# FofanovLab/mtsv_tools

Hardware: AMD Instinct MI355X
Metric: reads/sec (whole node), 150bp reads vs MG-index (higher is better)
Workload: dtype u32/i16

## Files before the change

### include/mtsv_amd.h

```cpp
#ifndef MTSV_AMD_H
#define MTSV_AMD_H

#include <stddef.h>
#include <stdint.h>

#ifdef __cplusplus
extern "C" {
#endif

#define MTSV_OK 0
#define MTSV_E_ARG (-1)
#define MTSV_E_IO (-2)
#define MTSV_E_FORMAT (-3)
#define MTSV_E_DEVICE (-4)
#define MTSV_E_LIMIT (-5)
#define MTSV_E_NOMEM (-6)

typedef struct mtsv_index mtsv_index;
typedef struct mtsv_batch mtsv_batch;

typedef struct {
    double edit_rate;
    uint32_t seed_size;
    uint32_t seed_interval;
// ... 21 lines not shown
    uint64_t sa_s;
    uint64_t file_bytes;
    uint64_t device_bytes;
    uint32_t kmer_k;
    uint32_t sa_full;
} mtsv_index_info_t;

#define MTSV_N_STAGES 8
typedef struct {
    float stage_ms[MTSV_N_STAGES];
    uint64_t n_reads;
    uint64_t n_seed_slots;
    uint64_t n_seed_hits;
    uint64_t lf_steps;
    uint64_t n_candidates;
    uint64_t n_verified;
    uint64_t window_bytes;
    uint64_t n_hits;
    uint64_t n_passes;
    uint64_t n_rounds;
    uint64_t n_lanes;
    uint64_t sw_cell_pairs;
    float sw_prefilter_ms;
    float sw_sweep_ms;
    uint64_t n_sw_passed;
    float sw_diag_ms;
    float sw_bound_ms;
    float edit_ms;
    uint64_t myers_columns;
    uint64_t n_sw_bound_refuted;
    uint64_t verify_turns;
    uint64_t verify_lanes_max;
    uint64_t myers_grid_max;
} mtsv_batch_stats;

const char *mtsv_last_error(void);
const char *mtsv_version(void);
void mtsv_params_default(mtsv_params *p);

int mtsv_device_count(void);

int mtsv_index_load(const char *path, mtsv_index **out);
int mtsv_index_build(uint64_t n_seqs, const uint32_t *tax_ids, const uint32_t *gis,
                     const uint8_t *const *seqs, const uint64_t *seq_lens, uint32_t occ_k,
                     uint64_t sa_s, int n_threads, mtsv_index **out);
int mtsv_index_build_fasta(const char *fasta_path, uint32_t occ_k, uint64_t sa_s, int n_threads,
                           mtsv_index **out);
int mtsv_set_build_device(int hip_device);
int mtsv_index_write(const mtsv_index *ix, const char *path);
int mtsv_index_info(const mtsv_index *ix, mtsv_index_info_t *info);
void mtsv_index_free(mtsv_index *ix);

#define MTSV_DEV_DEFAULT 0u
#define MTSV_DEV_SAMPLED_SA_ONLY 1u
#define MTSV_DEV_NO_KMER_TABLE 2u
int mtsv_index_to_device(mtsv_index *ix, int hip_device, uint32_t flags);

int mtsv_bin_batch(mtsv_index *ix, int hip_device, const uint8_t *bases, const uint64_t *read_off,
                   uint64_t n_reads, const mtsv_params *params, mtsv_hit **hits, uint64_t *n_hits);
void mtsv_hits_free(mtsv_hit *hits);
void *mtsv_host_alloc(size_t bytes);
void mtsv_host_free(void *p);
int mtsv_host_register(void *p, size_t bytes);
int mtsv_host_unregister(void *p);
int mtsv_bin_batch_multi(mtsv_index *ix, const int *devices, int n_devices, const uint8_t *bases,
                         const uint64_t *read_off, uint64_t n_reads, const mtsv_params *params,
// ... 70 lines not shown
```

### mtsv_tools_amd/_lib.py

```python
import ctypes as C
import os

import numpy as np

_HERE = os.path.dirname(os.path.abspath(__file__))


def lib_path():
    return os.environ.get("MTSV_AMD_LIB") or os.path.join(_HERE, "libmtsv_amd.so")


class MtsvError(RuntimeError):
    def __init__(self, code, msg):
        super().__init__(f"mtsv error {code}: {msg}")
        self.code = code


E_ARG, E_IO, E_FORMAT, E_DEVICE, E_LIMIT, E_NOMEM = -1, -2, -3, -4, -5, -6
MATCH_OFF, MATCH_WITH_HITS, MATCH_ONLY = 0, 1, 2
KEEP_UNMATCHED, KEEP_MATCHED = 0, 1


class Params(C.Structure):
    _fields_ = [("edit_rate", C.c_double), ("seed_size", C.c_uint32), ("seed_interval", C.c_uint32),
                ("min_seed", C.c_double), ("max_hits", C.c_uint64), ("tune_max_hits", C.c_uint64),
                ("max_assignments", C.c_int64), ("max_candidates", C.c_int64)]


class IndexInfo(C.Structure):
    _fields_ = [("n", C.c_uint64), ("n_bins", C.c_uint64), ("occ_k", C.c_uint32),
                ("sa_s", C.c_uint64), ("file_bytes", C.c_uint64), ("device_bytes", C.c_uint64),
                ("kmer_k", C.c_uint32), ("sa_full", C.c_uint32)]


N_STAGES = 8
STAGE_NAMES = ("search", "thin_scan", "expand", "locate", "coalesce", "verify", "gather", "total")


class BatchStats(C.Structure):
    _fields_ = [("stage_ms", C.c_float * N_STAGES), ("n_reads", C.c_uint64),
                ("n_seed_slots", C.c_uint64), ("n_seed_hits", C.c_uint64), ("lf_steps", C.c_uint64),
                ("n_candidates", C.c_uint64), ("n_verified", C.c_uint64),
                ("window_bytes", C.c_uint64), ("n_hits", C.c_uint64), ("n_passes", C.c_uint64),
                ("n_rounds", C.c_uint64), ("n_lanes", C.c_uint64), ("sw_cell_pairs", C.c_uint64), ("sw_prefilter_ms", C.c_float),
                ("sw_sweep_ms", C.c_float), ("n_sw_passed", C.c_uint64), ("sw_diag_ms", C.c_float), ("sw_bound_ms", C.c_float),
                ("edit_ms", C.c_float), ("myers_columns", C.c_uint64), ("n_sw_bound_refuted", C.c_uint64),
                ("verify_turns", C.c_uint64), ("verify_lanes_max", C.c_uint64), ("myers_grid_max", C.c_uint64)]

    def as_dict(self):
        d = {n: (float(getattr(self, n)) if t is C.c_float else int(getattr(self, n))) for n, t in self._fields_[1:]}
        d["stage_ms"] = {STAGE_NAMES[i]: float(self.stage_ms[i]) for i in range(N_STAGES)}
        return d


HIT_DTYPE = np.dtype({"names": ["read", "tax_id", "gi", "edit", "strand", "offset"],
                      "formats": ["<u8", "<u4", "<u4", "<u4", "u1", "<u8"],
                      "offsets": [0, 8, 12, 16, 20, 24], "itemsize": 32})

TAXON_STATS_DTYPE = np.dtype({"names": ["tax_id", "only_hit", "only_best", "tied_best", "not_best"],
                              "formats": ["<u4", "<u8", "<u8", "<u8", "<u8"],
                              "offsets": [0, 8, 16, 24, 32], "itemsize": 40})

EXPORTS = [
    "mtsv_last_error", "mtsv_version", "mtsv_params_default", "mtsv_device_count",
    "mtsv_index_load", "mtsv_index_build", "mtsv_index_build_fasta", "mtsv_index_write",
    "mtsv_index_info", "mtsv_index_free", "mtsv_set_build_device", "mtsv_index_to_device", "mtsv_bin_batch",
    "mtsv_hits_free", "mtsv_batch_create", "mtsv_batch_upload", "mtsv_batch_run", "mtsv_batch_run_host", "mtsv_batch_run_host_parts",
    "mtsv_batch_stats_get", "mtsv_batch_set_verify_mode", "mtsv_batch_download", "mtsv_batch_free", "mtsv_format_results",
    "mtsv_free", "mtsv_synth_index", "mtsv_synth_reads", "mtsv_bin_batch_workspace_reads",
    "mtsv_bin_batch_multi", "mtsv_bin_batch_chunks", "mtsv_set_default_verify_mode",
    "mtsv_host_alloc", "mtsv_host_free", "mtsv_host_register", "mtsv_host_unregister",
    "mtsv_batch_create_lanes", "mtsv_batch_reserve_host", "mtsv_pack_bases", "mtsv_host_pack_threads",
    "mtsv_batch_set_taxa_report", "mtsv_batch_taxa_report", "mtsv_merge_taxa_reports", "mtsv_format_taxa_report",
    "mtsv_batch_set_match_flags", "mtsv_batch_match_flags",
    "mtsv_batch_take_reads", "mtsv_batch_read_map", "mtsv_batch_download_reads",
]

_lib = None


# ... 400 lines not shown
```

### mtsv_tools_amd/csrc/batch.hip

```cpp
#include <atomic>
#include <chrono>
#include <cmath>
#include <condition_variable>
#include <exception>
#include <mutex>
#include <thread>
#include <cstdio>
#include <cstdlib>
#include <cstring>
#include <stdexcept>
#include <vector>

#include "../../include/mtsv_amd.h"
#include "batch.hpp"
#include "kernels.hpp"

namespace mtsv {

namespace {
template <class F>
void parallel_ranges(uint64_t n, F f) {
    static const int max_nt = [] {
        const char* e = getenv("MTSV_COPY_THREADS");
        return e ? std::max(1, std::min(16, atoi(e))) : 4;
// ... 91 lines not shown
    const uint64_t ns = 2 * ws_reads;
    if (!parent) {
        dev_alloc(&d_bases, max_bases + 64, &bytes);
        dev_alloc(&d_read_off, max_reads + 1, &bytes);
        dev_alloc(&d_codes, max_bases + 64, &bytes);
    }
    dev_alloc(&d_strand_hits, ns + 1, &bytes);
    dev_alloc(&d_strand_nseeds, ns, &bytes);
    dev_alloc(&d_strand_off, ns + 1, &bytes);
    dev_alloc(&d_strand_ncand, ns, &bytes);
    dev_alloc(&d_strand_nout, ns + 1, &bytes);
    dev_alloc(&d_heavy_list, 2 * ns, &bytes);
    dev_alloc(&d_out_off, ns + 1, &bytes);
    dev_alloc(&d_tile_sums, (uint64_t)scan_tiles((uint32_t)ns) + 1, &bytes);
    dev_alloc(&d_counters, kCounters, &bytes);
    alloc_hit_workspace();
    dev_alloc(&d_hits, hits_cap, &bytes);
    HIP_CHECK(hipHostMalloc((void**)&h_counters, kCounters * sizeof(uint64_t), hipHostMallocMapped));
    if (const char* e = getenv("MTSV_SW")) sw_pairs = strcmp(e, "packed") != 0;
    if (const char* e = getenv("MTSV_SW_DIAG")) sw_diag = atoi(e) != 0;
    if (const char* e = getenv("MTSV_SW_PREPASS")) sw_prepass = atoi(e) != 0;
    if (const char* e = getenv("MTSV_SW_TOP")) sw_top = atoi(e) != 0;
    if (const char* e = getenv("MTSV_SW_BOUND")) sw_bound = atoi(e) != 0;
    if (const char* e = getenv("MTSV_SW_FUSED")) sw_fused = atoi(e) != 0;
    verify_mode = g_default_verify_mode;
    if (const char* e = getenv("MTSV_VERIFY")) verify_mode = !strcmp(e, "edit_first") ? 1 : 0;
    if (!parent) {
        myers_wgs_per_cu = n_lanes > 1 ? kMyersWgsPerCuLanes : kMyersWgsPerCuMax;
        if (const char* e = getenv("MTSV_MYERS_WGS_PER_CU")) myers_wgs_per_cu = (uint32_t)std::max(1, std::min((int)kMyersWgsPerCuMax, atoi(e)));
        verify_turn.on = n_lanes > 1;
        if (const char* e = getenv("MTSV_VERIFY_TURN")) verify_turn.on = verify_turn.on && atoi(e) != 0;
        if (const char* e = getenv("MTSV_TAIL_FROM_LIST")) tail_from_list = atoi(e) != 0;
        if (const char* e = getenv("MTSV_FUSED_CLEAR")) fused_clear = atoi(e) != 0;
    } else {
        myers_wgs_per_cu = parent->myers_wgs_per_cu;
        tail_from_list = parent->tail_from_list;
        fused_clear = parent->fused_clear;
    }
    for (auto& e : ev) HIP_CHECK(hipEventCreate(&e));
    for (int k = 1; k < n_lanes; k++) {
        extra.emplace_back(new Batch(ix, di, ws_reads, 0, hit_cap_user, this));
        bytes += extra.back()->bytes;
    }
}

Batch::~Batch() {
    extra.clear();
    (void)hipSetDevice(di->device);
    (void)hipStreamSynchronize(stream);
    for (void* p : {(void*)d_bases, (void*)d_read_off, (void*)d_seed_lo, (void*)d_seed_cnt, (void*)d_seed_pre, (void*)d_strand_hits,
                    (void*)d_strand_nseeds, (void*)d_strand_off, (void*)d_strand_ncand, (void*)d_worklist,
                    (void*)d_strand_nout, (void*)d_out_off, (void*)d_tile_sums, (void*)d_counters, (void*)d_hit_row,
                    (void*)d_hit_ref, (void*)d_hit_q, (void*)d_hit_key, (void*)d_cand_tmp, (void*)d_cand, (void*)d_out,
                    (void*)d_hits, (void*)d_cand_next, (void*)d_cand_status, (void*)d_heavy_list})
        (void)hipFree(p);
    (void)hipFree(d_codes);
    (void)hipFree(d_strip);
    (void)hipFree(d_planes);
    (void)hipFree(report.d_taxa);
    (void)hipFree(report.d_counts);
    for (auto& e : report_ev)
        if (e) (void)hipEventDestroy(e);
    (void)hipFree(match.d_words);
    for (auto& e : match_ev)
        if (e) (void)hipEventDestroy(e);
    (void)hipFree(d_read_map);
    (void)hipFree(d_compact);
    for (auto& e : compact_ev)
        if (e) (void)hipEventDestroy(e);
    if (h_hits_stage) pinned_hits_release(h_hits_stage);
// ... 158 lines not shown
        l->reset_lane();
    }
    if (match.mode != MTSV_MATCH_OFF) {
        const uint64_t need = (n_reads + 63) / 64;
        if (need > match.cap_words || !match.d_words) {
            (void)hipFree(match.d_words);
            match.d_words = nullptr;
            match.cap_words = 0;
            uint64_t b = 0;
            dev_alloc(&match.d_words, need + need / 16 + 1, &b);
            match.cap_words = need + need / 16;
        }
        match.n_reads = n_reads;
        match.call_base = read_base;
        match.ms = 0;
        match.launches = 0;
        HIP_CHECK(hipMemsetAsync(match.d_words, 0, (match.cap_words + 1) * sizeof(uint64_t), stream));
        HIP_CHECK(hipStreamSynchronize(stream));
    }
}

void Batch::end_run() {
    finish_lane();
    for (auto& l : extra) l->finish_lane();
    const double wall_ms = (now_s() - run_t0) * 1e3;
    bool overlapped = false;
    for (auto& l : extra) {
        if (l->stats.n_passes == 0) continue;
        overlapped = true;
        for (int s = 0; s < 7; s++) stage_acc[s] += l->stage_acc[s];
        stats.n_seed_slots += l->stats.n_seed_slots;
        stats.n_seed_hits += l->stats.n_seed_hits;
        stats.n_passes += l->stats.n_passes;
        stats.n_rounds = std::max(stats.n_rounds, l->stats.n_rounds);
        stats.lf_steps += l->stats.lf_steps;
        stats.n_candidates += l->stats.n_candidates;
        stats.n_verified += l->stats.n_verified;
        stats.window_bytes += l->stats.window_bytes;
        stats.sw_cell_pairs += l->stats.sw_cell_pairs;
        stats.sw_prefilter_ms += l->stats.sw_prefilter_ms;
        stats.sw_sweep_ms += l->stats.sw_sweep_ms;
        stats.sw_diag_ms += l->stats.sw_diag_ms;
        stats.sw_bound_ms += l->stats.sw_bound_ms;
        stats.edit_ms += l->stats.edit_ms;
        stats.myers_columns += l->stats.myers_columns;
        stats.n_sw_bound_refuted += l->stats.n_sw_bound_refuted;
        stats.n_sw_passed += l->stats.n_sw_passed;
    }
    if (overlapped) stage_acc[7] = (float)wall_ms;
    for (int s = 0; s < MTSV_N_STAGES; s++) stats.stage_ms[s] = stage_acc[s];
    stats.n_reads = n_reads;
    stats.n_lanes = lanes_used;
    stats.verify_turns = verify_turn.taken;
    stats.verify_lanes_max = verify_turn.max_in_verify;
    stats.myers_grid_max = verify_turn.myers_grid_max;
    total_hits = 0;
    for (auto& sg : segments) total_hits += sg.count;
    stats.n_hits = total_hits;
}

void Batch::set_taxa_report(bool on) {
    if (parent) throw std::runtime_error("internal: the taxa report belongs to the workspace's owner");
    if (on && match.mode == MTSV_MATCH_ONLY)
        throw std::runtime_error("arg: the taxa report reads gathered hits and MTSV_MATCH_ONLY gathers none (mtsv_batch_set_match_flags)");
    if (on && !report.d_counts) {
        std::vector<uint32_t>& t = report.h_taxa;
// ... 287 lines not shown
        const uint32_t nstr = nr * 2;
        const uint64_t slots = (uint64_t)nstr * max_ns;
        if (slots > seed_cap) {
            (void)hipFree(d_seed_lo);
            (void)hipFree(d_seed_cnt);
            (void)hipFree(d_seed_pre);
            d_seed_lo = d_seed_cnt = d_seed_pre = nullptr;
            const uint64_t want = tiled ? slots : std::max<uint64_t>(slots, 2 * ws_reads * (uint64_t)max_ns);
            uint64_t dummy = 0;
            if (getenv("MTSV_TRACE")) fprintf(stderr, "[workspace] seed slot arrays grow %llu -> %llu entries\n", (unsigned long long)seed_cap, (unsigned long long)want);
            dev_alloc(&d_seed_lo, want, &dummy);
            dev_alloc(&d_seed_cnt, want, &dummy);
            dev_alloc(&d_seed_pre, want, &dummy);
            seed_cap = want;
        }
        const bool edit_first_path = !tiled && verify_mode == 1 && pass_max_len <= 253;
        const bool rounds_path = !tiled && !edit_first_path && sw_pairs && pass_max_len <= 253 && hit_cap < 0x80000000ull;
        const bool myers_pass = edit_first_path || rounds_path;
        const uint32_t plane_words = myers_pass ? myers_words(pass_max_len) : 0;
        if ((uint64_t)nr * 3 * plane_words > plane_cap) {
            (void)hipFree(d_planes);
            d_planes = nullptr;
            const uint64_t want = std::max<uint64_t>(nr, ws_reads) * 3 * plane_words;
            uint64_t dummy = 0;
            dev_alloc(&d_planes, want, &dummy);
            plane_cap = want;
        }
        HIP_CHECK(hipEventRecord(ev[0], stream));
        const uint32_t listed_cap = (uint32_t)std::min<uint64_t>(slots, std::max<uint64_t>(4096, (uint64_t)((double)slots * listed_share)));
        launch_search(stream, v, sb, so, (uint32_t)r0, nr, max_ns, K, G, d_seed_lo, d_seed_cnt, d_seed_pre, (uint32_t*)(d_counters + 22), listed_cap, di->d_kmer_levels,
                      fused_clear && ctr22_zero);
        ctr22_zero = false;
        HIP_CHECK(hipEventRecord(ev[1], stream));
        if (max_ns)
            launch_thin(stream, sb, so, (uint32_t)r0, nr, p.edit_rate, p.min_seed, max_ns, K, G, p.max_hits, p.tune_max_hits, d_seed_cnt,
                        d_seed_pre, d_strand_hits, d_strand_nseeds, myers_pass ? d_planes : nullptr, plane_words);
        else {
            HIP_CHECK(hipMemsetAsync(d_strand_hits, 0, (uint64_t)nstr * 4, stream));
            HIP_CHECK(hipMemsetAsync(d_strand_nseeds, 0, (uint64_t)nstr * 4, stream));
        }
        launch_scan(stream, d_strand_hits, nstr, d_tile_sums, d_counters + 0, d_strand_off);
        launch_publish(stream, d_counters, h_counters, 1);
        launch_publish(stream, d_counters + 22, h_counters + 22, 1);
        HIP_CHECK(hipEventRecord(ev[2], stream));
        HIP_CHECK(hipStreamSynchronize(stream));
        {
            const uint64_t n_listed = h_counters[22] & 0xffffffffull;
            const double share = slots ? (double)n_listed / (double)slots : 0.0;
            if (n_listed > listed_cap) {
                listed_share = std::min(1.0, share * 1.25 + 0.01);
                if (getenv("MTSV_TRACE")) fprintf(stderr, "[lane] %llu listed seed slots, grid for %u: pass again\n", (unsigned long long)n_listed, listed_cap);
                continue;
            }
            listed_share = std::min(1.0, std::max(0.02, share * 1.5 + 0.005));
        }
        const uint64_t total_hits = h_counters[0];
        if (total_hits > hit_cap) {
            if (nr > 1) {
                pass_reads = std::max<uint64_t>(1, nr / 2);
                continue;
            }
            if (total_hits > 0xfffffff0ull)
                throw std::runtime_error("device: one read has " + std::to_string(total_hits) + " seed hits, more than 2^32");
            grow_hit_workspace(total_hits);
        }
        stats.n_passes++;
        stats.n_seed_slots += slots;
        stats.n_seed_hits += total_hits;
        launch_expand(stream, v, nstr, max_ns, G, d_seed_lo, d_seed_cnt, d_seed_pre, d_strand_off, d_hit_row, d_hit_ref,
                      d_hit_q);
        HIP_CHECK(hipEventRecord(ev[3], stream));
        if (!v.sa_full)
            launch_locate(stream, v, (uint32_t)total_hits, d_strand_off + nstr, d_hit_row, d_hit_ref,
                          (unsigned long long*)(d_counters + 2));
        HIP_CHECK(hipEventRecord(ev[4], stream));
        if (fused_clear) {
            uint64_t mask = 1ull << 1 | 1ull << 7 | 1ull << 15 | 1ull << kCtrHeavyTicket | 1ull << 22;
            if (rounds_path) mask |= 1ull << 8 | 1ull << 9 | 1ull << 10 | 1ull << 11 | 1ull << 17 | 1ull << 18;
            launch_clear_counters(stream, d_counters, mask);
            ctr22_zero = true;
        } else {
            HIP_CHECK(hipMemsetAsync(d_counters + 1, 0, 8, stream));
            HIP_CHECK(hipMemsetAsync(d_counters + 7, 0, 8, stream));
            HIP_CHECK(hipMemsetAsync(d_counters + 15, 0, 8, stream));
        }
        launch_coalesce(stream, v, so, (uint32_t)r0, nstr, p.max_candidates, d_strand_off,
                        d_strand_nseeds, d_hit_ref, d_hit_q, d_hit_key, d_cand_tmp, d_cand, d_cand_next,
                        d_cand_status, d_strand_ncand, d_worklist, d_heavy_list, d_counters, fused_clear);
        HIP_CHECK(hipEventRecord(ev[5], stream));
        Batch* const root = parent ? parent : this;
        VerifyTurn::Guard turn;
        if (total_hits) turn.take(root->verify_turn, read_base + r0, this);
        const uint32_t R = root->myers_wgs_per_cu;
        {
            EvalArgs a;
            a.bases = sb;
            a.read_off = so;
            a.r0 = (uint32_t)r0;
            a.edit_rate = p.edit_rate;
            a.max_candidates = p.max_candidates;
            a.strand_off = d_strand_off;
            a.cand = d_cand;
            a.cand_next = d_cand_next;
// ... 807 lines not shown
```

### mtsv_tools_amd/csrc/batch.hpp

```cpp
#pragma once
#include <condition_variable>
#include <memory>
#include <mutex>
#include <vector>

#include "../../include/mtsv_amd.h"
#include "host_pack.hpp"
#include "dev_index.hpp"
#include "kernels.hpp"

namespace mtsv {

struct Batch {
    mtsv_index* ix;
    DeviceIndex* di;
    hipStream_t stream = nullptr, copy_stream2 = nullptr;
    mtsv_hit* h_hits_stage = nullptr;
    uint64_t h_hits_cap = 0, staged_hits = 0, last_total_hits = 0;
    bool staged_valid = false;
    struct Arena {
        uint8_t* d_bases = nullptr;
        uint8_t* d_packed = nullptr;
        uint32_t* d_off = nullptr;
        uint64_t cap_bases = 0, cap_reads = 0;
// ... 29 lines not shown
    uint32_t *d_seed_lo = nullptr, *d_seed_cnt = nullptr, *d_seed_pre = nullptr;
    uint64_t seed_cap = 0;
    uint32_t *d_strand_hits = nullptr, *d_strand_nseeds = nullptr, *d_strand_off = nullptr, *d_strand_ncand = nullptr,
             *d_worklist = nullptr, *d_strand_nout = nullptr, *d_out_off = nullptr;
    uint64_t* d_tile_sums = nullptr;
    uint64_t* d_counters = nullptr;
    uint32_t *d_hit_row = nullptr, *d_hit_ref = nullptr, *d_hit_q = nullptr;
    uint64_t *d_hit_key = nullptr, *d_cand_tmp = nullptr;
    uint4 *d_cand = nullptr, *d_out = nullptr;
    uint32_t *d_cand_next = nullptr, *d_cand_status = nullptr, *d_heavy_list = nullptr;
    DevHit* d_hits = nullptr;
    uint2* d_strip = nullptr;
    uint64_t strip_cap = 0;
    uint32_t* d_planes = nullptr;
    uint64_t plane_cap = 0;
    uint64_t* h_counters = nullptr;
    hipEvent_t ev[15];
    float sw_ms_acc = 0, sweep_ms_acc = 0, diag_ms_acc = 0, bound_ms_acc = 0, edit_ms_acc = 0;
    uint64_t sw_passed_acc = 0;

    std::vector<uint32_t> h_read_off;
    uint32_t max_len = 0;
    static constexpr int kCounters = 25;
    double listed_share = 0.125;
    bool sw_diag = true;
    bool sw_top = true;
    bool sw_bound = true;
    bool sw_fused = true;
    bool sw_prepass = true;
    bool sw_pairs = true;
    uint32_t myers_wgs_per_cu = kMyersWgsPerCuMax;
    bool tail_from_list = true;
    bool fused_clear = true;
    bool ctr22_zero = false;
    struct VerifyTurn {
        bool on = false;
        std::mutex mu;
        std::condition_variable cv;
        bool held = false;
        std::vector<std::pair<uint64_t, const Batch*>> waiting;
        uint64_t taken = 0, in_verify = 0, max_in_verify = 0, myers_grid_max = 0;
        void enter(uint64_t first_read, const Batch* lane);
        void leave();
        void note_grid(uint32_t blocks);
        struct Guard {
            VerifyTurn* t = nullptr;
            Guard() = default;
            Guard(const Guard&) = delete;
            Guard& operator=(const Guard&) = delete;
            ~Guard() { release(); }
            void take(VerifyTurn& turn, uint64_t first_read, const Batch* lane) {
                if (t) return;
                turn.enter(first_read, lane);
                t = &turn;
            }
            void release() {
                if (t) t->leave();
                t = nullptr;
            }
        };
    };
    VerifyTurn verify_turn;
    int verify_mode = 0;
    uint64_t n_reads = 0;
    uint64_t n_hits_total = 0;
    mtsv_batch_stats stats{};
// ... 100 lines not shown
```

### mtsv_tools_amd/csrc/k_seed.hip

```cpp
#include "kernels_common.hpp"

namespace mtsv {

namespace {

__device__ inline uint32_t fast_code(uint32_t ch);
__global__ __launch_bounds__(256) void k_normalise(const uint8_t* src, uint8_t* dst, uint64_t lo, uint64_t hi) {
    const uint64_t i = (lo & ~15ull) + ((uint64_t)blockIdx.x * blockDim.x + threadIdx.x) * 16;
    if (i >= hi) return;
    if (i < lo || i + 16 > hi) {
        const uint64_t a = i < lo ? lo : i, b = i + 16 > hi ? hi : i + 16;
        for (uint64_t q = a; q < b; q++) dst[q] = (uint8_t)fast_code(src[q]);
        return;
    }
    uint4 v = *reinterpret_cast<const uint4*>(src + i);
    uint32_t w[4] = {v.x, v.y, v.z, v.w};
#pragma unroll
    for (int k = 0; k < 4; k++) {
        uint32_t o = 0;
#pragma unroll
        for (int q = 0; q < 4; q++) o |= fast_code((w[k] >> (8 * q)) & 0xffu) << (8 * q);
        w[k] = o;
    }
    *reinterpret_cast<uint4*>(dst + i) = make_uint4(w[0], w[1], w[2], w[3]);
// ... 451 lines not shown
                const uint32_t o01 = (uint32_t)__builtin_amdgcn_update_dpp(0, (int)h01, 0xB1, 0xf, 0xf, false);
                const uint32_t on = (uint32_t)__builtin_amdgcn_update_dpp(0, (int)hn, 0xB1, 0xf, 0xf, false);
                const uint32_t lo01 = half ? o01 : h01, hi01 = half ? h01 : o01;
                const uint32_t c0 = (lo01 & 0xffffu) | (hi01 << 16), c1 = (lo01 >> 16) | (hi01 & 0xffff0000u);
                const uint32_t cn = half ? (on | (hn << 16)) : (hn | (on << 16));
                if (i && ((i - 1) & 1) == half) {
                    const uint32_t w = i - 1, left = L - 32 * w;
                    const uint32_t m = left >= 32 ? 0xffffffffu : (1u << left) - 1u;
                    const uint32_t w0 = __builtin_amdgcn_alignbit(c0, a0, sh) & m, w1 = __builtin_amdgcn_alignbit(c1, a1, sh) & m,
                                   wn = __builtin_amdgcn_alignbit(cn, an, sh) & m;
                    nn += __popc(wn);
                    if (img) {
                        img[3 * w] = w0;
                        img[3 * w + 1] = w1;
                        img[3 * w + 2] = wn;
                    }
                }
                a0 = c0;
                a1 = c1;
                an = cn;
              }
            }
        }
        nn += (uint32_t)__shfl_xor((int)nn, 1);
        hopeless = hopeless || nn > ED;
        const double ms = floor((double)nseeds * min_seed);
        const uint32_t min_seeds = ms < 1.0 ? 1u : (ms > 65535.0 ? 65535u : (uint32_t)ms);
        nseeds = min_seeds | (ED << 16) | ((need && hopeless) ? kHopeless : 0u);
    }
    strand_hits[rs] = total;
    strand_nseeds[rs] = nseeds;
}

constexpr int kScanThreads = 256;
constexpr int kScanItems = 8;
constexpr int kScanTile = kScanThreads * kScanItems;

__device__ inline uint32_t wave_incl_scan(uint32_t v) {
    for (int d = 1; d < kWave; d <<= 1) {
        uint32_t o = __shfl_up(v, d);
        if ((int)lane_id() >= d) v += o;
    }
    return v;
}

__global__ __launch_bounds__(kScanThreads) void k_scan_tile_sums(const uint32_t* __restrict__ in, uint32_t n,
                                                                 uint64_t* __restrict__ tile_sums) {
    __shared__ uint32_t ws[kScanThreads / kWave];
    uint32_t base = blockIdx.x * kScanTile + threadIdx.x * kScanItems;
    uint32_t s = 0;
    for (int i = 0; i < kScanItems; i++)
        if (base + i < n) s += in[base + i];
    for (int d = 32; d > 0; d >>= 1) s += __shfl_down(s, d);
    if (lane_id() == 0) ws[threadIdx.x / kWave] = s;
    __syncthreads();
    if (threadIdx.x == 0) {
        uint64_t t = 0;
        for (int w = 0; w < kScanThreads / kWave; w++) t += ws[w];
        tile_sums[blockIdx.x] = t;
    }
}

__global__ __launch_bounds__(1024) void k_scan_sums(uint64_t* __restrict__ tile_sums, uint32_t n_tiles,
                                                    uint64_t* __restrict__ total) {
    __shared__ uint64_t buf[1024];
    __shared__ uint64_t carry;
// ... 56 lines not shown
    const uint32_t raw = slot < n_slots ? seed_cnt[slot] : 0;
    const bool at_pos = raw == kSeedAtPos;
    const uint32_t c = at_pos ? 1u : raw;
    uint32_t o = 0, l = 0, q = 0;
    if (c) {
        const uint32_t rs = (uint32_t)(slot / max_ns), j = (uint32_t)(slot % max_ns);
        o = strand_off[rs] + seed_pre[slot];
        l = seed_lo[slot];
        q = j * G;
    }
    constexpr uint32_t kOwn = 16;
    if (at_pos) {
        hit_ref[o] = l;
        hit_q[o] = q;
    } else if (c && c <= kOwn) {
        for (uint32_t i = 0; i < c; i++) {
            if (ix.sa_full) hit_ref[o + i] = ix.sa_full[l + i];
            else hit_row[o + i] = l + i;
            hit_q[o + i] = q;
        }
    }
    unsigned long long big = __ballot(c > kOwn);
    const uint32_t lane = lane_id();
    while (big) {
        const int src = __ffsll((long long)big) - 1;
        big &= big - 1;
        const uint32_t cs = __builtin_amdgcn_readlane(c, src), os = __builtin_amdgcn_readlane(o, src);
        const uint32_t ls = __builtin_amdgcn_readlane(l, src), qs = __builtin_amdgcn_readlane(q, src);
        for (uint32_t i = lane; i < cs; i += kWave) {
            if (ix.sa_full) hit_ref[os + i] = ix.sa_full[ls + i];
            else hit_row[os + i] = ls + i;
            hit_q[os + i] = qs;
        }
    }
}

constexpr uint32_t kLocateChunk = 512;

__global__ __launch_bounds__(256) void k_locate(DevIndexView ix, const uint32_t* __restrict__ total_hits,
                                                const uint32_t* __restrict__ hit_row,
                                                uint32_t* __restrict__ hit_ref, unsigned long long* __restrict__ lf_steps) {
    const uint32_t total = *total_hits;
    const uint32_t lane = lane_id();
    const uint32_t wave = (blockIdx.x * blockDim.x + threadIdx.x) / kWave;
    const uint32_t n_waves = gridDim.x * blockDim.x / kWave;
    unsigned long long my_steps = 0;
    for (uint64_t cbase = (uint64_t)wave * kLocateChunk; cbase < total; cbase += (uint64_t)n_waves * kLocateChunk) {
        uint32_t next = (uint32_t)cbase;
        const uint32_t end = (uint32_t)min((uint64_t)total, cbase + kLocateChunk);
        bool active = false;
        uint32_t idx = 0, row = 0, steps = 0;
        for (;;) {
            unsigned long long need = __ballot(!active);
            uint32_t take = next + __popcll(need & ((1ull << lane) - 1));
            if (!active && take < end) {
                idx = take;
                row = hit_row[idx];
                steps = 0;
                active = true;
            }
            next += __popcll(need);
            if (!__any(active)) break;
            if (active) {
                bool sampled = ix.sa_pow2_shift != 0xffffffffu ? (row & (ix.sa_s - 1)) == 0 : (row % ix.sa_s) == 0;
                if (sampled) {
                    uint32_t j = ix.sa_pow2_shift != 0xffffffffu ? row >> ix.sa_pow2_shift : row / ix.sa_s;
// ... 65 lines not shown
    if (!fast) {
        hipLaunchKernelGGL(k_search, dim3(cdiv(total, 256)), dim3(256), 0, s, ix, bases, read_off, r0, n_reads, max_ns, K, G,
                           seed_lo, seed_cnt, kmer_levels);
        return;
    }
    const dim3 grid(std::min<uint32_t>(cdiv(total, 256), 256 * 16));
#define FAST_CASE(KKV)                                                                                                  \
    if (K - KKV > 2)                                                                                                    \
        hipLaunchKernelGGL((k_search_fast<KKV, true>), grid, dim3(256), 0, s, ix, bases, read_off, r0, (uint32_t)total, max_ns, K, G, \
                           seed_lo, seed_cnt, slow_list, slow_count);                                                   \
    else                                                                                                                \
        hipLaunchKernelGGL((k_search_fast<KKV, false>), grid, dim3(256), 0, s, ix, bases, read_off, r0, (uint32_t)total, max_ns, K, G, \
                           seed_lo, seed_cnt, slow_list, slow_count)
    switch (ix.kmer_k) {
    case 12: FAST_CASE(12); break;
    case 13: FAST_CASE(13); break;
    case 14: FAST_CASE(14); break;
    case 15: FAST_CASE(15); break;
    case 17: FAST_CASE(17); break;
    default: FAST_CASE(16); break;
    }
#undef FAST_CASE
    hipLaunchKernelGGL(k_search_listed, dim3(cdiv(std::max<uint32_t>(listed_cap, 1), 256)), dim3(256), 0, s, ix, bases, read_off, r0, max_ns, K, G,
                       slow_list, slow_count, seed_lo, seed_cnt, kmer_levels);
}

void launch_thin(hipStream_t s, const uint8_t* bases, const uint32_t* read_off, uint32_t r0, uint32_t n_reads, double edit_rate,
                 double min_seed, uint32_t max_ns, uint32_t K, uint32_t G, uint64_t max_hits, uint64_t tune, uint32_t* seed_cnt, uint32_t* seed_pre,
                 uint32_t* strand_hits, uint32_t* strand_nseeds, uint32_t* planes, uint32_t plane_words) {
    hipLaunchKernelGGL(k_thin, dim3(cdiv((uint64_t)n_reads * 2, 256)), dim3(256), 0, s, bases, read_off, r0, n_reads, edit_rate,
                       min_seed, max_ns, K, G, max_hits, tune, seed_cnt, seed_pre, strand_hits, strand_nseeds, planes, plane_words);
}

void launch_scan(hipStream_t s, const uint32_t* in, uint32_t n, uint64_t* tile_sums, uint64_t* total, uint32_t* out) {
    uint32_t tiles = cdiv(n ? n : 1, kScanTile);
    hipLaunchKernelGGL(k_scan_tile_sums, dim3(tiles), dim3(kScanThreads), 0, s, in, n, tile_sums);
    hipLaunchKernelGGL(k_scan_sums, dim3(1), dim3(1024), 0, s, tile_sums, tiles, total);
    hipLaunchKernelGGL(k_scan_apply, dim3(tiles), dim3(kScanThreads), 0, s, in, n, tile_sums, total, out);
}
uint32_t scan_tiles(uint32_t n) { return cdiv(n ? n : 1, kScanTile); }

void launch_expand(hipStream_t s, const DevIndexView& ix, uint32_t n_strands, uint32_t max_ns, uint32_t G,
                   const uint32_t* seed_lo, const uint32_t* seed_cnt, const uint32_t* seed_pre, const uint32_t* strand_off,
                   uint32_t* hit_row, uint32_t* hit_ref, uint32_t* hit_q) {
    uint64_t n_slots = (uint64_t)n_strands * max_ns;
    if (!n_slots) return;
    hipLaunchKernelGGL(k_expand, dim3(cdiv(n_slots, 256)), dim3(256), 0, s, ix, n_slots, max_ns, G, seed_lo, seed_cnt, seed_pre,
                       strand_off, hit_row, hit_ref, hit_q);
}

void launch_locate(hipStream_t s, const DevIndexView& ix, uint32_t total_hits_host, const uint32_t* total_hits_dev,
                   const uint32_t* hit_row, uint32_t* hit_ref, unsigned long long* lf_steps) {
    if (!total_hits_host) return;
    uint32_t chunks = cdiv(total_hits_host, kLocateChunk);
    uint32_t blocks = std::min<uint32_t>(cdiv(chunks, 4), 256 * 8);
    hipLaunchKernelGGL(k_locate, dim3(blocks), dim3(256), 0, s, ix, total_hits_dev, hit_row, hit_ref, lf_steps);
}

}
```

### mtsv_tools_amd/csrc/kernels.hpp

```cpp
#pragma once
#include <algorithm>

#include "dev_layout.hpp"

namespace mtsv {

struct DevHit {
    uint64_t read;
    uint32_t tax_id;
    uint32_t gi;
    uint32_t edit;
    uint8_t strand;
    uint8_t pad[3];
    uint64_t offset;
};
static_assert(sizeof(DevHit) == 32, "DevHit must match mtsv_hit");

constexpr uint32_t kCtrVerified = 4, kCtrWindowBytes = 5, kCtrSwCursor = 8, kCtrPassCount = 9, kCtrSwCellPairs = 14;
constexpr uint32_t kCtrHeavyWalk = 23, kCtrHeavyTicket = 24;

struct EvalArgs {
    const uint8_t* bases;
    const uint32_t* read_off;
    uint32_t r0;
// ... 14 lines not shown
    unsigned long long* window_bytes;
    unsigned long long* sw_columns = nullptr;
    uint32_t* pass_list = nullptr;
    uint32_t* pass_count = nullptr;
    uint32_t* next_list = nullptr;
    uint32_t* next_count = nullptr;
    unsigned long long* myers_ctr = nullptr;
    uint32_t* und_list = nullptr;
    uint32_t und_slot = 0;
    uint2* strip = nullptr;
    uint32_t strip_len = 0;
    const uint32_t* planes = nullptr;
    uint32_t plane_words = 0;
    uint32_t maxc = 0xffffffffu;
    uint32_t claim_shift = 0;
};

inline uint32_t myers_words(uint32_t max_len) { return std::min(std::max((max_len + 31) / 32, 2u), 8u); }

constexpr uint32_t kMaxRegisterReadLen = 256;
constexpr uint32_t kMaxReadLen = 32767;

void launch_publish(hipStream_t s, const uint64_t* src, uint64_t* dst_host, uint32_t n);
void launch_clear_counters(hipStream_t s, uint64_t* counters, uint64_t mask);
void launch_normalise(hipStream_t s, const uint8_t* src, uint8_t* dst, uint64_t begin, uint64_t end);
void launch_unpack(hipStream_t s, const uint8_t* packed, uint8_t* dst, uint64_t lo, uint64_t hi);
void launch_search(hipStream_t s, const DevIndexView& ix, const uint8_t* bases, const uint32_t* read_off, uint32_t r0,
                   uint32_t n_reads, uint32_t max_ns, uint32_t K, uint32_t G, uint32_t* seed_lo, uint32_t* seed_cnt,
                   uint32_t* slow_list, uint32_t* slow_count, uint32_t listed_cap, const uint2* kmer_levels,
                   bool count_is_zero = false);
void launch_thin(hipStream_t s, const uint8_t* bases, const uint32_t* read_off, uint32_t r0, uint32_t n_reads, double edit_rate,
                 double min_seed, uint32_t max_ns, uint32_t K, uint32_t G, uint64_t max_hits, uint64_t tune, uint32_t* seed_cnt, uint32_t* seed_pre,
                 uint32_t* strand_hits, uint32_t* strand_nseeds, uint32_t* planes, uint32_t plane_words);
void launch_scan(hipStream_t s, const uint32_t* in, uint32_t n, uint64_t* tile_sums, uint64_t* total, uint32_t* out);
uint32_t scan_tiles(uint32_t n);
void launch_expand(hipStream_t s, const DevIndexView& ix, uint32_t n_strands, uint32_t max_ns, uint32_t G,
                   const uint32_t* seed_lo, const uint32_t* seed_cnt, const uint32_t* seed_pre, const uint32_t* strand_off,
                   uint32_t* hit_row, uint32_t* hit_ref, uint32_t* hit_q);
void launch_locate(hipStream_t s, const DevIndexView& ix, uint32_t total_hits_host, const uint32_t* total_hits_dev,
                   const uint32_t* hit_row, uint32_t* hit_ref, unsigned long long* lf_steps);
void launch_coalesce(hipStream_t s, const DevIndexView& ix, const uint32_t* read_off, uint32_t r0, uint32_t n_strands,
                     int64_t max_candidates, const uint32_t* strand_off,
                     const uint32_t* strand_nseeds, const uint32_t* hit_ref, const uint32_t* hit_q, uint64_t* hit_key,
                     uint64_t* cand_tmp, uint4* cand, uint32_t* cand_next, uint32_t* cand_status,
                     uint32_t* strand_ncand, uint32_t* worklist, uint32_t* heavy_list, uint64_t* counters,
                     bool ticket_is_zero = false);
void launch_evaluate(hipStream_t s, const DevIndexView& ix, const EvalArgs& a, uint64_t max_items, uint32_t max_len);
void launch_evaluate_tiled(hipStream_t s, const DevIndexView& ix, const EvalArgs& a, uint64_t max_items);
uint32_t tiled_groups(uint64_t max_items, uint32_t strip_len);
void launch_max_window(hipStream_t s, uint32_t n_strands, const uint32_t* strand_off, const uint32_t* strand_ncand,
                       const uint4* cand, unsigned long long* out);
constexpr uint32_t kMyersWgsPerCuMax = 5;
uint32_t launch_edit_myers(hipStream_t s, const DevIndexView& ix, const EvalArgs& a, uint64_t max_items, uint32_t max_len,
                           int mode = 0, uint32_t wgs_per_cu = kMyersWgsPerCuMax, bool listed = false);
void launch_sw_pairs(hipStream_t s, const DevIndexView& ix, const EvalArgs& a, uint64_t max_items, uint32_t max_len,
                     bool diag = true, bool top = false, bool sparse = false);
void launch_sw_diag(hipStream_t s, const DevIndexView& ix, const EvalArgs& a, uint64_t max_items, uint32_t max_len,
                    uint32_t* sweep_list, uint32_t sweep_slot);
void launch_resolve(hipStream_t s, uint32_t n_strands, int64_t max_candidates, int64_t max_assignments,
                    const uint32_t* strand_off, const uint32_t* strand_ncand, const uint32_t* cand_status, uint4* out,
                    uint32_t* strand_nout);
void launch_gather(hipStream_t s, uint32_t n_strands, uint64_t r0, const uint32_t* strand_off, const uint32_t* strand_nout,
                   const uint32_t* out_off, const uint4* out, DevHit* hits, uint64_t hits_base);
constexpr uint32_t kReportDenseTaxa = 4095;
constexpr uint32_t kReportHashSlots = 4096;
void launch_report(hipStream_t s, uint32_t n_reads, const uint32_t* strand_nout, const uint32_t* out_off, const DevHit* hits,
// ... 13 lines not shown
```

Before: 432.4 million.

## Add tiled seed-thinning and expand kernels using LDS staging and wave-local prefix

Adds a tiled thinning kernel that stages 128 reads' seed counts and packed base bit-planes in shared memory, and an expand kernel that computes per-slot hit offsets with an in-wave prefix over a halo of seed counts. Together they drop the per-slot seed_pre prefix array. Expand also software-prefetches the next tile and splits small and large seed ranges between flat and wave-wide writes. The new path is on by default when max_ns is at most 16 and reads fit the register length, with an environment variable to fall back to the old path. A trace print and a stats counter are added too. The risks are correctness of the halo-based prefix and higher shared-memory use per block.

```diff
diff --git a/include/mtsv_amd.h b/include/mtsv_amd.h
--- a/include/mtsv_amd.h
+++ b/include/mtsv_amd.h
@@ -77,6 +77,7 @@
     uint64_t verify_turns;
     uint64_t verify_lanes_max;
     uint64_t myers_grid_max;
+    uint64_t n_seed_tile_passes;
 } mtsv_batch_stats;
 
 const char *mtsv_last_error(void);
diff --git a/mtsv_tools_amd/_lib.py b/mtsv_tools_amd/_lib.py
--- a/mtsv_tools_amd/_lib.py
+++ b/mtsv_tools_amd/_lib.py
@@ -45,7 +45,8 @@
                 ("n_rounds", C.c_uint64), ("n_lanes", C.c_uint64), ("sw_cell_pairs", C.c_uint64), ("sw_prefilter_ms", C.c_float),
                 ("sw_sweep_ms", C.c_float), ("n_sw_passed", C.c_uint64), ("sw_diag_ms", C.c_float), ("sw_bound_ms", C.c_float),
                 ("edit_ms", C.c_float), ("myers_columns", C.c_uint64), ("n_sw_bound_refuted", C.c_uint64),
-                ("verify_turns", C.c_uint64), ("verify_lanes_max", C.c_uint64), ("myers_grid_max", C.c_uint64)]
+                ("verify_turns", C.c_uint64), ("verify_lanes_max", C.c_uint64), ("myers_grid_max", C.c_uint64),
+                ("n_seed_tile_passes", C.c_uint64)]
 
     def as_dict(self):
         d = {n: (float(getattr(self, n)) if t is C.c_float else int(getattr(self, n))) for n, t in self._fields_[1:]}
diff --git a/mtsv_tools_amd/csrc/batch.hip b/mtsv_tools_amd/csrc/batch.hip
--- a/mtsv_tools_amd/csrc/batch.hip
+++ b/mtsv_tools_amd/csrc/batch.hip
@@ -147,10 +147,12 @@
         if (const char* e = getenv("MTSV_VERIFY_TURN")) verify_turn.on = verify_turn.on && atoi(e) != 0;
         if (const char* e = getenv("MTSV_TAIL_FROM_LIST")) tail_from_list = atoi(e) != 0;
         if (const char* e = getenv("MTSV_FUSED_CLEAR")) fused_clear = atoi(e) != 0;
+        if (const char* e = getenv("MTSV_SEED_STAGE")) seed_tiles = strcmp(e, "legacy") != 0;
     } else {
         myers_wgs_per_cu = parent->myers_wgs_per_cu;
         tail_from_list = parent->tail_from_list;
         fused_clear = parent->fused_clear;
+        seed_tiles = parent->seed_tiles;
     }
     for (auto& e : ev) HIP_CHECK(hipEventCreate(&e));
     for (int k = 1; k < n_lanes; k++) {
@@ -375,6 +377,7 @@
         stats.n_seed_slots += l->stats.n_seed_slots;
         stats.n_seed_hits += l->stats.n_seed_hits;
         stats.n_passes += l->stats.n_passes;
+        stats.n_seed_tile_passes += l->stats.n_seed_tile_passes;
         stats.n_rounds = std::max(stats.n_rounds, l->stats.n_rounds);
         stats.lf_steps += l->stats.lf_steps;
         stats.n_candidates += l->stats.n_candidates;
@@ -728,7 +731,11 @@
                       fused_clear && ctr22_zero);
         ctr22_zero = false;
         HIP_CHECK(hipEventRecord(ev[1], stream));
-        if (max_ns)
+        const bool tile_pass = seed_tiles && max_ns && seed_tile_fits(max_ns, pass_max_len, slots);
+        if (tile_pass)
+            launch_thin_tiled(stream, sb, so, (uint32_t)r0, nr, p.edit_rate, p.min_seed, max_ns, K, G, p.max_hits, p.tune_max_hits, d_seed_cnt,
+                              d_strand_hits, d_strand_nseeds, myers_pass ? d_planes : nullptr, plane_words);
+        else if (max_ns)
             launch_thin(stream, sb, so, (uint32_t)r0, nr, p.edit_rate, p.min_seed, max_ns, K, G, p.max_hits, p.tune_max_hits, d_seed_cnt,
                         d_seed_pre, d_strand_hits, d_strand_nseeds, myers_pass ? d_planes : nullptr, plane_words);
         else {
@@ -761,10 +768,15 @@
             grow_hit_workspace(total_hits);
         }
         stats.n_passes++;
+        stats.n_seed_tile_passes += tile_pass;
+        if (getenv("MTSV_TRACE")) fprintf(stderr, "[lane] pass of %u reads, max_ns %u, longest read %u: seed stage %s\n", nr, max_ns, pass_max_len, tile_pass ? "by tiles" : "legacy");
         stats.n_seed_slots += slots;
         stats.n_seed_hits += total_hits;
-        launch_expand(stream, v, nstr, max_ns, G, d_seed_lo, d_seed_cnt, d_seed_pre, d_strand_off, d_hit_row, d_hit_ref,
-                      d_hit_q);
+        if (tile_pass)
+            launch_expand_tiled(stream, v, nstr, max_ns, G, d_seed_lo, d_seed_cnt, d_strand_off, d_hit_row, d_hit_ref, d_hit_q);
+        else
+            launch_expand(stream, v, nstr, max_ns, G, d_seed_lo, d_seed_cnt, d_seed_pre, d_strand_off, d_hit_row, d_hit_ref,
+                          d_hit_q);
         HIP_CHECK(hipEventRecord(ev[3], stream));
         if (!v.sa_full)
             launch_locate(stream, v, (uint32_t)total_hits, d_strand_off + nstr, d_hit_row, d_hit_ref,
diff --git a/mtsv_tools_amd/csrc/batch.hpp b/mtsv_tools_amd/csrc/batch.hpp
--- a/mtsv_tools_amd/csrc/batch.hpp
+++ b/mtsv_tools_amd/csrc/batch.hpp
@@ -85,6 +85,7 @@
     uint32_t myers_wgs_per_cu = kMyersWgsPerCuMax;
     bool tail_from_list = true;
     bool fused_clear = true;
+    bool seed_tiles = true;
     bool ctr22_zero = false;
     struct VerifyTurn {
         bool on = false;
diff --git a/mtsv_tools_amd/csrc/k_seed.hip b/mtsv_tools_amd/csrc/k_seed.hip
--- a/mtsv_tools_amd/csrc/k_seed.hip
+++ b/mtsv_tools_amd/csrc/k_seed.hip
@@ -507,6 +507,124 @@
     strand_nseeds[rs] = nseeds;
 }
 
+constexpr uint32_t kThinTile = 128;
+constexpr uint32_t kTileMaxNs = 16;
+constexpr uint32_t kTilePitch = kTileMaxNs | 1;
+constexpr uint32_t kTileMaxWords = kMaxRegisterReadLen / 32;
+constexpr uint32_t kThinStreamWords = (kThinTile * kMaxRegisterReadLen + 32) / 32 + 2;
+
+__global__ __launch_bounds__(256) void k_thin_tiled(const uint8_t* __restrict__ bases, const uint32_t* __restrict__ read_off,
+                                                    uint32_t r0, uint32_t n_reads, double edit_rate, double min_seed,
+                                                    uint32_t max_ns, uint32_t K, uint32_t G, uint64_t max_hits,
+                                                    uint64_t tune_max_hits, uint32_t* __restrict__ seed_cnt,
+                                                    uint32_t* __restrict__ strand_hits, uint32_t* __restrict__ strand_nseeds,
+                                                    uint32_t* __restrict__ planes, uint32_t plane_words) {
+    __shared__ uint32_t s_off[kThinTile + 1];
+    __shared__ uint32_t s_cnt[2 * kThinTile * kTilePitch];
+    __shared__ uint32_t s_bits[3][kThinStreamWords];
+    __shared__ uint32_t s_need[kThinTile];
+    __shared__ uint32_t s_nn[kThinTile];
+    const uint32_t tid = threadIdx.x;
+    const uint32_t t0 = blockIdx.x * kThinTile, tn = min(kThinTile, n_reads - t0);
+    for (uint32_t i = tid; i <= tn; i += 256) s_off[i] = read_off[r0 + t0 + i];
+    if (tid < kThinTile) s_nn[tid] = 0;
+    __syncthreads();
+    const uint32_t pitch = max_ns | 1;
+    {
+        const uint32_t n_cnt = 2 * tn * max_ns;
+        const uint32_t* gc = seed_cnt + (uint64_t)2 * t0 * max_ns;
+        for (uint32_t e = tid; e < n_cnt; e += 256) {
+            const uint32_t row = e / max_ns;
+            s_cnt[row * pitch + (e - row * max_ns)] = gc[e];
+        }
+    }
+    const uint32_t g0 = s_off[0] >> 4;
+    {
+        const uint4* b128 = reinterpret_cast<const uint4*>(bases);
+        const uint32_t ng = min(((s_off[tn] + 15) >> 4) - g0, 2 * (kThinStreamWords - 1));
+        uint16_t* h0 = reinterpret_cast<uint16_t*>(s_bits[0]);
+        uint16_t* h1 = reinterpret_cast<uint16_t*>(s_bits[1]);
+        uint16_t* hn = reinterpret_cast<uint16_t*>(s_bits[2]);
+        for (uint32_t g = tid; g < ng; g += 256) {
+            const uint4 v = b128[g0 + g];
+            const uint32_t c0 = (v.x & 0x07070707u) | ((v.y & 0x07070707u) << 4);
+            const uint32_t c1 = (v.z & 0x07070707u) | ((v.w & 0x07070707u) << 4);
+            auto gather = [](uint32_t y) {
+                y &= 0x11111111u;
+                y |= y >> 7;
+                y |= y >> 14;
+                return y & 0xffu;
+            };
+            h0[g] = (uint16_t)(gather(c0) | (gather(c1) << 8));
+            h1[g] = (uint16_t)(gather(c0 >> 1) | (gather(c1 >> 1) << 8));
+            hn[g] = (uint16_t)(gather(c0 >> 2) | (gather(c1 >> 2) << 8));
+        }
+    }
+    __syncthreads();
+    const bool strand_lane = tid < 2 * tn;
+    uint32_t L = 0, total = 0, nseeds = 0;
+    if (strand_lane) {
+        L = s_off[(tid >> 1) + 1] - s_off[tid >> 1];
+        const uint32_t ns = n_seeds_of(L, K, G);
+        uint64_t next_offset = 0, seed_interval = G;
+        const uint32_t* cnt = s_cnt + tid * pitch;
+        uint32_t* gcnt = seed_cnt + ((uint64_t)2 * t0 + tid) * max_ns;
+        for (uint32_t j = 0; j < ns; j++) {
+            uint64_t offset = (uint64_t)j * G;
+            const uint32_t raw = cnt[j];
+            const uint32_t c = raw == kSeedAtPos ? 1u : raw;
+            if (offset < next_offset) {
+                if (c) gcnt[j] = 0;
+                continue;
+            }
+            if (c == 0) continue;
+            if ((uint64_t)c > max_hits) {
+                gcnt[j] = 0;
+                continue;
+            }
+            if ((uint64_t)c > tune_max_hits) {
+                seed_interval *= 2;
+                next_offset = offset + seed_interval;
+            }
+            total += c;
+            nseeds++;
+        }
+    }
+    const bool need = total != 0;
+    {
+        const int other_need = __shfl_xor((int)need, 1);
+        if (strand_lane && !(tid & 1)) s_need[tid >> 1] = need || other_need != 0;
+    }
+    __syncthreads();
+    for (uint32_t e = tid; e < tn * kTileMaxWords; e += 256) {
+        const uint32_t t = e / kTileMaxWords, w = e % kTileMaxWords;
+        const uint32_t b0 = s_off[t], Lt = s_off[t + 1] - b0;
+        if (!s_need[t] || w >= ((Lt + 31) >> 5)) continue;
+        const uint32_t bp = b0 - (g0 << 4) + 32 * w;
+        const uint32_t wi = min(bp >> 5, kThinStreamWords - 2), sh = bp & 31u;
+        const uint32_t left = Lt - 32 * w;
+        const uint32_t m = left >= 32 ? 0xffffffffu : (1u << left) - 1u;
+        const uint32_t w0 = __builtin_amdgcn_alignbit(s_bits[0][wi + 1], s_bits[0][wi], sh) & m;
+        const uint32_t w1 = __builtin_amdgcn_alignbit(s_bits[1][wi + 1], s_bits[1][wi], sh) & m;
+        const uint32_t wn = __builtin_amdgcn_alignbit(s_bits[2][wi + 1], s_bits[2][wi], sh) & m;
+        if (wn) atomicAdd(&s_nn[t], (uint32_t)__popc(wn));
+        if (planes) {
+            uint32_t* img = planes + ((uint64_t)(t0 + t) * plane_words + w) * 3;
+            img[0] = w0;
+            img[1] = w1;
+            img[2] = wn;
+        }
+    }
+    __syncthreads();
+    if (!strand_lane) return;
+    const uint32_t ED = (uint32_t)ceil((double)L * edit_rate);
+    const bool hopeless = 2ull * ED > (uint64_t)L || s_nn[tid >> 1] > ED;
+    const double ms = floor((double)nseeds * min_seed);
+    const uint32_t min_seeds = ms < 1.0 ? 1u : (ms > 65535.0 ? 65535u : (uint32_t)ms);
+    strand_hits[2 * t0 + tid] = total;
+    strand_nseeds[2 * t0 + tid] = min_seeds | (ED << 16) | ((need && hopeless) ? kHopeless : 0u);
+}
+
 constexpr int kScanThreads = 256;
 constexpr int kScanItems = 8;
 constexpr int kScanTile = kScanThreads * kScanItems;
@@ -629,6 +747,100 @@
             else hit_row[os + i] = ls + i;
             hit_q[os + i] = qs;
         }
+    }
+}
+
+__global__ __launch_bounds__(256) void k_expand_tiled(DevIndexView ix, uint32_t n_slots, uint32_t max_ns, uint32_t G,
+                                                      const uint32_t* __restrict__ seed_lo,
+                                                      const uint32_t* __restrict__ seed_cnt,
+                                                      const uint32_t* __restrict__ strand_off,
+                                                      uint32_t* __restrict__ hit_row, uint32_t* __restrict__ hit_ref,
+                                                      uint32_t* __restrict__ hit_q) {
+    __shared__ uint32_t stage[256 / kWave][kTileMaxNs + kWave];
+    __shared__ uint32_t flat[256 / kWave][4][kWave];
+    const uint32_t lane = lane_id(), wave = threadIdx.x / kWave;
+    uint32_t* st = stage[wave];
+    uint32_t (*fl)[kWave] = flat[wave];
+    const uint32_t n_tiles = (n_slots + kWave - 1) / kWave;
+    const uint32_t stride = gridDim.x * (256 / kWave);
+    struct Ahead {
+        uint32_t raw, halo, lo, off;
+    };
+    auto load_ahead = [&](uint32_t tile) {
+        Ahead a{0, 0, 0, 0};
+        const uint32_t base = tile * kWave, slot = base + lane;
+        if (tile < n_tiles && slot < n_slots) {
+            a.raw = seed_cnt[slot];
+            a.lo = seed_lo[slot];
+            a.off = strand_off[slot / max_ns];
+        }
+        const uint32_t back = kTileMaxNs - lane;
+        if (tile < n_tiles && lane < kTileMaxNs && back < max_ns && back <= base) a.halo = seed_cnt[base - back];
+        return a;
+    };
+    uint32_t tile = blockIdx.x * (256 / kWave) + wave;
+    Ahead next = load_ahead(tile);
+    for (; tile < n_tiles; tile += stride) {
+        const uint32_t slot = tile * kWave + lane;
+        const Ahead cur = next;
+        next = load_ahead(tile + stride);
+        const uint32_t raw = cur.raw, halo = cur.halo;
+        const bool at_pos = raw == kSeedAtPos;
+        const uint32_t c = at_pos ? 1u : raw;
+        st[kTileMaxNs + lane] = c;
+        if (lane < kTileMaxNs) st[lane] = halo == kSeedAtPos ? 1u : halo;
+        __builtin_amdgcn_fence(__ATOMIC_SEQ_CST, "wavefront");
+        __builtin_amdgcn_wave_barrier();
+        uint32_t o = 0, l = 0, q = 0;
+        if (c) {
+            const uint32_t rs = slot / max_ns, j = slot - rs * max_ns;
+            uint32_t pre = 0;
+            for (uint32_t i = 1; i <= j; i++) pre += st[kTileMaxNs + lane - i];
+            o = cur.off + pre;
+            l = cur.lo;
+            q = j * G;
+        }
+        constexpr uint32_t kOwn = 16;
+        if (at_pos) {
+            hit_ref[o] = l;
+            hit_q[o] = q;
+        }
+        const uint32_t cc = !at_pos && c <= kOwn ? c : 0;
+        const uint32_t inc = wave_incl_scan(cc);
+        const uint32_t sum = __builtin_amdgcn_readlane(inc, kWave - 1);
+        if (sum) {
+            fl[0][lane] = inc;
+            fl[1][lane] = o;
+            fl[2][lane] = l;
+            fl[3][lane] = q;
+            __builtin_amdgcn_fence(__ATOMIC_SEQ_CST, "wavefront");
+            __builtin_amdgcn_wave_barrier();
+            for (uint32_t f = lane; f < sum; f += kWave) {
+                uint32_t src = 0;
+#pragma unroll
+                for (uint32_t step = kWave / 2; step; step >>= 1)
+                    if (fl[0][src + step - 1] <= f) src += step;
+                const uint32_t i = f - (src ? fl[0][src - 1] : 0u);
+                const uint32_t os = fl[1][src], ls = fl[2][src];
+                if (ix.sa_full) hit_ref[os + i] = ix.sa_full[ls + i];
+                else hit_row[os + i] = ls + i;
+                hit_q[os + i] = fl[3][src];
+            }
+        }
+        unsigned long long big = __ballot(c > kOwn);
+        while (big) {
+            const int src = __ffsll((long long)big) - 1;
+            big &= big - 1;
+            const uint32_t cs = __builtin_amdgcn_readlane(c, src), os = __builtin_amdgcn_readlane(o, src);
+            const uint32_t ls = __builtin_amdgcn_readlane(l, src), qs = __builtin_amdgcn_readlane(q, src);
+            for (uint32_t i = lane; i < cs; i += kWave) {
+                if (ix.sa_full) hit_ref[os + i] = ix.sa_full[ls + i];
+                else hit_row[os + i] = ls + i;
+                hit_q[os + i] = qs;
+            }
+        }
+        __builtin_amdgcn_fence(__ATOMIC_SEQ_CST, "wavefront");
+        __builtin_amdgcn_wave_barrier();
     }
 }
 
@@ -760,6 +972,29 @@
                        min_seed, max_ns, K, G, max_hits, tune, seed_cnt, seed_pre, strand_hits, strand_nseeds, planes, plane_words);
 }
 
+bool seed_tile_fits(uint32_t max_ns, uint32_t max_len, uint64_t n_slots) {
+    return max_ns <= kTileMaxNs && max_len <= kMaxRegisterReadLen && n_slots <= 0xffffff00ull;
+}
+uint32_t seed_tile_reads() { return kThinTile; }
+uint32_t seed_tile_max_ns() { return kTileMaxNs; }
+
+void launch_thin_tiled(hipStream_t s, const uint8_t* bases, const uint32_t* read_off, uint32_t r0, uint32_t n_reads, double edit_rate,
+                       double min_seed, uint32_t max_ns, uint32_t K, uint32_t G, uint64_t max_hits, uint64_t tune, uint32_t* seed_cnt,
+                       uint32_t* strand_hits, uint32_t* strand_nseeds, uint32_t* planes, uint32_t plane_words) {
+    if (!n_reads) return;
+    hipLaunchKernelGGL(k_thin_tiled, dim3(cdiv(n_reads, kThinTile)), dim3(256), 0, s, bases, read_off, r0, n_reads, edit_rate, min_seed,
+                       max_ns, K, G, max_hits, tune, seed_cnt, strand_hits, strand_nseeds, planes, plane_words);
+}
+
+void launch_expand_tiled(hipStream_t s, const DevIndexView& ix, uint32_t n_strands, uint32_t max_ns, uint32_t G, const uint32_t* seed_lo,
+                         const uint32_t* seed_cnt, const uint32_t* strand_off, uint32_t* hit_row, uint32_t* hit_ref, uint32_t* hit_q) {
+    const uint64_t n_slots = (uint64_t)n_strands * max_ns;
+    if (!n_slots) return;
+    const dim3 grid(std::min<uint32_t>(cdiv(n_slots, 256), 256 * 8));
+    hipLaunchKernelGGL(k_expand_tiled, grid, dim3(256), 0, s, ix, (uint32_t)n_slots, max_ns, G, seed_lo, seed_cnt, strand_off, hit_row,
+                       hit_ref, hit_q);
+}
+
 void launch_scan(hipStream_t s, const uint32_t* in, uint32_t n, uint64_t* tile_sums, uint64_t* total, uint32_t* out) {
     uint32_t tiles = cdiv(n ? n : 1, kScanTile);
     hipLaunchKernelGGL(k_scan_tile_sums, dim3(tiles), dim3(kScanThreads), 0, s, in, n, tile_sums);
diff --git a/mtsv_tools_amd/csrc/kernels.hpp b/mtsv_tools_amd/csrc/kernels.hpp
--- a/mtsv_tools_amd/csrc/kernels.hpp
+++ b/mtsv_tools_amd/csrc/kernels.hpp
@@ -70,6 +70,14 @@
 void launch_thin(hipStream_t s, const uint8_t* bases, const uint32_t* read_off, uint32_t r0, uint32_t n_reads, double edit_rate,
                  double min_seed, uint32_t max_ns, uint32_t K, uint32_t G, uint64_t max_hits, uint64_t tune, uint32_t* seed_cnt, uint32_t* seed_pre,
                  uint32_t* strand_hits, uint32_t* strand_nseeds, uint32_t* planes, uint32_t plane_words);
+bool seed_tile_fits(uint32_t max_ns, uint32_t max_len, uint64_t n_slots);
+uint32_t seed_tile_reads();
+uint32_t seed_tile_max_ns();
+void launch_thin_tiled(hipStream_t s, const uint8_t* bases, const uint32_t* read_off, uint32_t r0, uint32_t n_reads, double edit_rate,
+                       double min_seed, uint32_t max_ns, uint32_t K, uint32_t G, uint64_t max_hits, uint64_t tune, uint32_t* seed_cnt,
+                       uint32_t* strand_hits, uint32_t* strand_nseeds, uint32_t* planes, uint32_t plane_words);
+void launch_expand_tiled(hipStream_t s, const DevIndexView& ix, uint32_t n_strands, uint32_t max_ns, uint32_t G, const uint32_t* seed_lo,
+                         const uint32_t* seed_cnt, const uint32_t* strand_off, uint32_t* hit_row, uint32_t* hit_ref, uint32_t* hit_q);
 void launch_scan(hipStream_t s, const uint32_t* in, uint32_t n, uint64_t* tile_sums, uint64_t* total, uint32_t* out);
 uint32_t scan_tiles(uint32_t n);
 void launch_expand(hipStream_t s, const DevIndexView& ix, uint32_t n_strands, uint32_t max_ns, uint32_t G,
```

New measurement: 442.8 million, median of 6. +2.4%, better.
